# wwang2/CoarseGrainingVAE

Hardware: NVIDIA B200
Metric: conformations/s (fwd+bwd train step) (higher is better)
Workload: dtype f32

## Files before the change

### coarsegrainingvae_b200/_lib.py

```python
import ctypes
import os
import re

_HERE = os.path.dirname(os.path.abspath(__file__))
LIB_PATH = os.path.join(_HERE, "libcgvae_sm100.so")
HEADER_PATH = os.path.join(_HERE, "..", "include", "cgvae_b200.h")

_lib = None

_P = ctypes.c_void_p
_I64 = ctypes.c_int64
_INT = ctypes.c_int
_F32 = ctypes.c_float
_SZ = ctypes.c_size_t

SIGNATURES = {
    "cgvae_abi_version": (_INT, []),
    "cgvae_last_error": (ctypes.c_char_p, []),
    "cgvae_launch_count": (ctypes.c_ulonglong, []),
    "cgvae_set_error_flags": (_INT, [_INT, _P]),
    "cgvae_radius_graph_ws_bytes": (_SZ, [_I64, _I64]),
    "cgvae_radius_graph_count": (_INT, [_P, _I64, _P, _I64, _F32, _INT, _INT, _P, _P, _SZ, _P]),
    "cgvae_radius_graph_fill": (_INT, [_P, _I64, _P, _I64, _F32, _INT, _INT, _P, _P, _P, _SZ, _P]),
    "cgvae_exclusive_scan": (_INT, [_P, _I64, _P, _P]),
# ... 24 lines not shown
                                  _P, _P, _P, _P, _P, _P, _P, _P, _P, _P, _P]),
    "cgvae_update_norm_fwd": (_INT, [_P, _P, _I64, _INT, _P, _P]),
    "cgvae_update_combine_fwd": (_INT, [_P, _P, _P, _P, _P, _I64, _INT, _INT, _P, _P, _P]),
    "cgvae_update_combine_bwd": (_INT, [_P, _P, _P, _P, _P, _I64, _INT, _P, _P, _P, _P]),
    "cgvae_update_norm_bwd": (_INT, [_P, _P, _P, _P, _I64, _INT, _INT, _P, _P, _P]),
    "cgvae_update_combine_bwd_ld": (_INT, [_P, _P, _P, _P, _P, _I64, _INT, _P, _P, _P, _I64, _P]),
    "cgvae_update_norm_bwd_ld": (_INT, [_P, _P, _P, _P, _I64, _INT, _INT, _P, _P, _I64, _P]),
    "cgvae_segment_reduce_fwd": (_INT, [_P, _P, _P, _I64, _I64, _INT, _P, _P]),
    "cgvae_segment_reduce_bwd": (_INT, [_P, _P, _P, _I64, _I64, _INT, _P, _P]),
    "cgvae_gather_rows": (_INT, [_P, _P, _I64, _I64, _I64, _P, _P]),
    "cgvae_lift_fwd": (_INT, [_P, _P, _P, _P, _P, _P, _P, _I64, _I64, _INT, _INT, _P, _P]),
    "cgvae_lift_bwd": (_INT, [_P, _P, _P, _P, _P, _P, _I64, _I64, _INT, _INT, _P, _P]),
    "cgvae_adam_ws_bytes": (_SZ, []),
    "cgvae_adam_clip_step": (_INT, [_P, _P, _P, _P, _I64, _F32, _F32, _F32, _F32, _F32, _F32, _P, _P, _P, _F32, _F32, _P,
                                    _P, _SZ, _P]),
    "cgvae_bond_graph": (_INT, [_P, _P, _I64, _F32, _P, _P]),
    "cgvae_sample_quality": (_INT, [_P, _P, _P, _P, _I64, _I64, _F32, _P, _P, _P]),
    "cgvae_set_pdl": (_INT, [_INT]),
    "cgvae_set_matmul_precision": (_INT, [_INT]),
    "cgvae_get_matmul_precision": (_INT, []),
    "cgvae_register_const_range": (_INT, [_P, _SZ]),
    "cgvae_grad_sumsq": (_INT, [_P, _I64, _P, _P, _SZ, _P]),
    "cgvae_adam_apply": (_INT, [_P, _P, _P, _P, _I64, _F32, _F32, _F32, _F32, _F32, _F32, _P, _P, _INT, _F32, _F32, _P, _P, _SZ, _P]),
    "cgvae_dihedral_loss_fwd": (_INT, [_P, _P, _P, _I64, _P, _P, _P, _P, _P, _SZ, _P]),
    "cgvae_dihedral_loss_bwd": (_INT, [_P, _P, _P, _P, _I64, _I64, _P, _P, _P, _P]),
    "cgvae_pin_mask": (_INT, [_P, _I64, _P, _I64, _P, _SZ, _P]),
    "cgvae_vae_latent_fwd": (_INT, [_P, _P, _P, _I64, _P, _P, _P]),
    "cgvae_vae_latent_bwd": (_INT, [_P, _P, _P, _P, _I64, _P, _P, _P]),
    "cgvae_std_logvar_fwd": (_INT, [_P, _I64, _F32, _P, _P]),
    "cgvae_std_logvar_bwd": (_INT, [_P, _P, _I64, _F32, _P, _P]),
# ... 47 lines not shown
```

### coarsegrainingvae_b200/csrc/optim.cu

```cuda
#include "common.cuh"

namespace cgvae {

constexpr int kNormBlocks = 1024;

__global__ void __launch_bounds__(256) sumsq_partial_kernel(const float* __restrict__ g, int64_t n, float* __restrict__ partial,
                                                            unsigned int* __restrict__ ticket) {
  CGVAE_KERNEL_PROLOGUE();
  __shared__ float red[8];
  const int64_t per = (n + kNormBlocks - 1) / kNormBlocks;
  const int64_t beg = (int64_t)blockIdx.x * per, end = min(n, beg + per);
  float s = 0.f;
  for (int64_t i = beg + threadIdx.x; i < end; i += 256) {
    const float x = g[i];
    s = fmaf(x, x, s);
  }
  s = warp_sum(s);
  if ((threadIdx.x & 31) == 0) red[threadIdx.x >> 5] = s;
  __syncthreads();
  if (threadIdx.x == 0) {
    float t = 0.f;
#pragma unroll
    for (int w = 0; w < 8; ++w) t += red[w];
    partial[blockIdx.x] = t;
// ... 66 lines not shown
        const float gg = g[j] * coef;
        const float mm = beta1 * m[j] + (1.0f - beta1) * gg;
        const float vv = beta2 * v[j] + (1.0f - beta2) * gg * gg;
        m[j] = mm; v[j] = vv;
        p[j] -= step_size * mm / (sqrtf(vv) * inv_sqrt_bc2 + eps);
      }
    }
  }
  __syncthreads();
  if (threadIdx.x == 0) {
    __threadfence();
    if (atomicAdd(ticket, 1u) == gridDim.x - 1) step[0] = t;
  }
}

}

using namespace cgvae;

extern "C" {

size_t cgvae_adam_ws_bytes(void) { return sizeof(float) * (kNormBlocks + 4); }

int cgvae_adam_clip_step(float* p, const float* g, float* m, float* v, int64_t n, float max_norm, float grad_scale, float lr,
                         float beta1, float beta2, float eps, float* step, float* norm_out, const float* loss,
                         float loss_scale, float loss_limit, float* skipped, void* ws, size_t ws_bytes,
                         cgvae_stream_t stream) {
  if (n == 0) return 0;
  CGVAE_REQUIRE(p && g && m && v && step && ws && ws_bytes >= cgvae_adam_ws_bytes(), "adam_clip_step: bad arguments");
  CGVAE_REQUIRE(aligned16(p) && aligned16(g) && aligned16(m) && aligned16(v), "adam_clip_step: buffers must be 16-byte aligned");
// ... 21 lines not shown
int cgvae_adam_apply(float* p, const float* g, float* m, float* v, int64_t n, float max_norm, float grad_scale, float lr, float beta1,
                     float beta2, float eps, float* step, float* norm_out, int use_ws_loss, float loss_scale, float loss_limit,
                     float* skipped, void* ws, size_t ws_bytes, cgvae_stream_t stream) {
  if (n == 0) return 0;
  CGVAE_REQUIRE(p && g && m && v && step && ws && ws_bytes >= cgvae_adam_ws_bytes(), "adam_apply: bad arguments");
  CGVAE_REQUIRE(aligned16(p) && aligned16(g) && aligned16(m) && aligned16(v), "adam_apply: buffers must be 16-byte aligned");
  float* partial = reinterpret_cast<float*>(ws);
  unsigned int* ticket = reinterpret_cast<unsigned int*>(partial + kNormBlocks + 1);
  const unsigned blocks = (unsigned)std::min<int64_t>(ceil_div(n, 256 * 4), 148 * 8);
  launch_kernel(adam_clip_kernel, dim3(blocks), dim3(256), 0, (cudaStream_t)stream, p, g, m, v, n, (const float*)partial, max_norm, grad_scale, lr,
                beta1, beta2, eps, step, norm_out, use_ws_loss ? (const float*)(partial + kNormBlocks) : (const float*)nullptr, loss_scale,
                loss_limit, skipped, ticket);
  return launched("adam_clip");
}

}
```

### coarsegrainingvae_b200/csrc/wgrad.cu

```cuda
#include "common.cuh"

namespace cgvae {

constexpr int WG_MAXP = 48;
constexpr int WG_ROWS = 32;
constexpr int WG_T = 64;
constexpr int WG_STRIP = 4;
constexpr int WG_FAST_ROWS = 16;

struct WgradBatch {
  cgvae_wgrad_problem p[WG_MAXP];
  int tile_begin[WG_MAXP + 1];
  int n;
};
static_assert(sizeof(WgradBatch) <= 4000, "problem table must fit the 4 KB kernel parameter space");

__device__ __forceinline__ void stage_rows(float (*dst)[WG_T], const float* __restrict__ src, int ld, int r0, int rows,
                                           int c0, int ncols, bool vec, int tid, int seg_rows, int64_t seg_stride) {
  const int rn = min(WG_ROWS, rows - r0);
  for (int idx = tid; idx < rn * (WG_T / 4); idx += 256) {
    const int r = idx / (WG_T / 4), c = 4 * (idx % (WG_T / 4));
    float4 val = make_float4(0.f, 0.f, 0.f, 0.f);
    {
      const int R = r0 + r;
      const float* q;
      if (seg_rows > 0) {
        const int sgm = R / seg_rows;
        q = src + (int64_t)sgm * seg_stride + (int64_t)(R - sgm * seg_rows) * ld + c0 + c;
      } else {
        q = src + (int64_t)R * ld + c0 + c;
      }
      if (vec && c0 + c + 3 < ncols) {
        val = __ldg(reinterpret_cast<const float4*>(q));
      } else {
        if (c0 + c + 0 < ncols) val.x = __ldg(q + 0);
        if (c0 + c + 1 < ncols) val.y = __ldg(q + 1);
        if (c0 + c + 2 < ncols) val.z = __ldg(q + 2);
        if (c0 + c + 3 < ncols) val.w = __ldg(q + 3);
      }
    }
    *reinterpret_cast<float4*>(&dst[r][c]) = val;
  }
}

__global__ void __launch_bounds__(256) wgrad_grouped_kernel(const __grid_constant__ WgradBatch batch) {
  CGVAE_KERNEL_PROLOGUE();
  __shared__ __align__(16) float gs[WG_ROWS][WG_T];
  __shared__ __align__(16) float xs[WG_ROWS][WG_T];
  const int tid = threadIdx.x, bid = blockIdx.x;
  int lo = 0, hi = batch.n;
  while (hi - lo > 1) {
    const int mid = (lo + hi) >> 1;
    if (batch.tile_begin[mid] <= bid) lo = mid; else hi = mid;
  }
  const cgvae_wgrad_problem& P = batch.p[lo];
  const float* __restrict__ gy = P.gy;
  const float* __restrict__ x = P.x;
  float* __restrict__ dW = P.dW;
  float* __restrict__ db = P.db;
  const int rows = P.rows, n_out = P.n_out, n_in = P.n_in, ldg = P.ldg, ldx = P.ldx, seg_rows = P.seg_rows;
  const int64_t sg = P.seg_stride_g, sx = P.seg_stride_x;
  const bool has_w = (dW != nullptr);
  const int strips_k = has_w ? (n_in + WG_STRIP * WG_T - 1) / (WG_STRIP * WG_T) : 1;
  const int t = bid - batch.tile_begin[lo];
  const int n0 = (t / strips_k) * WG_T, kstrip = (t % strips_k) * WG_STRIP * WG_T;
  const bool g_vec = ((reinterpret_cast<uintptr_t>(gy) & 15) == 0) && (ldg % 4 == 0) && (seg_rows == 0 || sg % 4 == 0);
  const bool x_vec = has_w && ((reinterpret_cast<uintptr_t>(x) & 15) == 0) && (ldx % 4 == 0) && (seg_rows == 0 || sx % 4 == 0);
  const bool w_vec = has_w && ((reinterpret_cast<uintptr_t>(dW) & 15) == 0) && (n_in % 4 == 0);
  const int ty = tid >> 4, tx = tid & 15;
  const bool one_chunk = rows <= WG_ROWS;

  if (one_chunk) stage_rows(gs, gy, ldg, 0, rows, n0, n_out, g_vec, tid, seg_rows, sg);
  if (db != nullptr && kstrip == 0) {
    float bsum = 0.f;
    for (int r0 = 0; r0 < rows; r0 += WG_ROWS) {
      if (!one_chunk) {
        __syncthreads();
        stage_rows(gs, gy, ldg, r0, rows, n0, n_out, g_vec, tid, seg_rows, sg);
      }
      __syncthreads();
      const int rn = min(WG_ROWS, rows - r0);
      if (tid < WG_T)
        for (int r = 0; r < rn; ++r) bsum += gs[r][tid];
    }
    if (tid < WG_T && n0 + tid < n_out) db[n0 + tid] = bsum;
  }
  if (!has_w) return;
  if (rows <= WG_FAST_ROWS) {
    __shared__ __align__(16) float xw[WG_FAST_ROWS][WG_STRIP * WG_T];
    const int ncol4 = WG_STRIP * WG_T / 4;
    for (int idx = tid; idx < rows * ncol4; idx += 256) {
      const int r = idx / ncol4, c = 4 * (idx % ncol4);
      float4 val = make_float4(0.f, 0.f, 0.f, 0.f);
      const float* q;
      if (seg_rows > 0) {
        const int sgm = r / seg_rows;
        q = x + (int64_t)sgm * sx + (int64_t)(r - sgm * seg_rows) * ldx + kstrip + c;
      } else {
        q = x + (int64_t)r * ldx + kstrip + c;
      }
      if (x_vec && kstrip + c + 3 < n_in) {
        val = __ldg(reinterpret_cast<const float4*>(q));
      } else {
        if (kstrip + c + 0 < n_in) val.x = __ldg(q + 0);
        if (kstrip + c + 1 < n_in) val.y = __ldg(q + 1);
        if (kstrip + c + 2 < n_in) val.z = __ldg(q + 2);
        if (kstrip + c + 3 < n_in) val.w = __ldg(q + 3);
      }
      *reinterpret_cast<float4*>(&xw[r][c]) = val;
    }
    __syncthreads();
#pragma unroll
    for (int kk = 0; kk < WG_STRIP; ++kk) {
      const int k0 = kstrip + kk * WG_T;
      if (k0 >= n_in) break;
      float acc[4][4];
#pragma unroll
      for (int a = 0; a < 4; ++a)
#pragma unroll
        for (int b = 0; b < 4; ++b) acc[a][b] = 0.f;
      for (int r = 0; r < rows; ++r) {
        const float4 g4 = *reinterpret_cast<const float4*>(&gs[r][4 * ty]);
        const float4 x4 = *reinterpret_cast<const float4*>(&xw[r][kk * WG_T + 4 * tx]);
        const float g[4] = {g4.x, g4.y, g4.z, g4.w}, xv[4] = {x4.x, x4.y, x4.z, x4.w};
#pragma unroll
        for (int a = 0; a < 4; ++a)
#pragma unroll
          for (int b = 0; b < 4; ++b) acc[a][b] = fmaf(g[a], xv[b], acc[a][b]);
      }
      const int k = k0 + 4 * tx;
#pragma unroll
      for (int a = 0; a < 4; ++a) {
        const int n = n0 + 4 * ty + a;
        if (n >= n_out) continue;
        float* dst = dW + (int64_t)n * n_in + k;
        if (w_vec && k + 3 < n_in) {
          *reinterpret_cast<float4*>(dst) = make_float4(acc[a][0], acc[a][1], acc[a][2], acc[a][3]);
        } else {
#pragma unroll
          for (int b = 0; b < 4; ++b)
            if (k + b < n_in) dst[b] = acc[a][b];
        }
      }
    }
    return;
  }
  for (int kk = 0; kk < WG_STRIP; ++kk) {
    const int k0 = kstrip + kk * WG_T;
    if (k0 >= n_in) break;
    float acc[4][4];
#pragma unroll
    for (int a = 0; a < 4; ++a)
#pragma unroll
      for (int b = 0; b < 4; ++b) acc[a][b] = 0.f;
    for (int r0 = 0; r0 < rows; r0 += WG_ROWS) {
      __syncthreads();
      if (!one_chunk) stage_rows(gs, gy, ldg, r0, rows, n0, n_out, g_vec, tid, seg_rows, sg);
      stage_rows(xs, x, ldx, r0, rows, k0, n_in, x_vec, tid, seg_rows, sx);
      __syncthreads();
      const int rn = min(WG_ROWS, rows - r0);
#pragma unroll 4
      for (int r = 0; r < rn; ++r) {
        const float4 g4 = *reinterpret_cast<const float4*>(&gs[r][4 * ty]);
        const float4 x4 = *reinterpret_cast<const float4*>(&xs[r][4 * tx]);
        const float g[4] = {g4.x, g4.y, g4.z, g4.w}, xv[4] = {x4.x, x4.y, x4.z, x4.w};
#pragma unroll
        for (int a = 0; a < 4; ++a)
#pragma unroll
          for (int b = 0; b < 4; ++b) acc[a][b] = fmaf(g[a], xv[b], acc[a][b]);
      }
    }
    const int k = k0 + 4 * tx;
#pragma unroll
    for (int a = 0; a < 4; ++a) {
      const int n = n0 + 4 * ty + a;
      if (n >= n_out) continue;
      float* dst = dW + (int64_t)n * n_in + k;
      if (w_vec && k + 3 < n_in) {
        *reinterpret_cast<float4*>(dst) = make_float4(acc[a][0], acc[a][1], acc[a][2], acc[a][3]);
      } else {
#pragma unroll
        for (int b = 0; b < 4; ++b)
          if (k + b < n_in) dst[b] = acc[a][b];
      }
    }
  }
}

}

using namespace cgvae;

extern "C" {

int cgvae_wgrad_grouped(const cgvae_wgrad_problem* problems, int n_problems, cgvae_stream_t stream) {
  CGVAE_REQUIRE(n_problems >= 0, "wgrad_grouped: negative problem count");
  if (n_problems == 0) return 0;
  CGVAE_REQUIRE(problems != nullptr, "wgrad_grouped: null problem table");
  for (int i = 0; i < n_problems; ++i) {
    const cgvae_wgrad_problem& q = problems[i];
    CGVAE_REQUIRE(q.gy && (q.dW || q.db), "wgrad_grouped: problem %d has no operand / no output", i);
    CGVAE_REQUIRE(!q.dW || q.x, "wgrad_grouped: problem %d: dW without x", i);
    CGVAE_REQUIRE(q.rows >= 0 && q.n_out >= 1 && q.ldg >= q.n_out, "wgrad_grouped: problem %d: bad gy shape", i);
    CGVAE_REQUIRE(!q.dW || (q.n_in >= 1 && q.ldx >= q.n_in), "wgrad_grouped: problem %d: bad x shape", i);
    CGVAE_REQUIRE(q.seg_rows >= 0 && (q.seg_rows == 0 || q.rows % q.seg_rows == 0),
                  "wgrad_grouped: problem %d: rows must be a multiple of seg_rows", i);
  }
  cudaStream_t st = (cudaStream_t)stream;
  for (int base = 0; base < n_problems; base += WG_MAXP) {
    WgradBatch batch;
    batch.n = std::min(WG_MAXP, n_problems - base);
    int64_t tiles = 0;
    for (int i = 0; i < batch.n; ++i) {
      batch.p[i] = problems[base + i];
      batch.tile_begin[i] = (int)tiles;
      const cgvae_wgrad_problem& q = batch.p[i];
      tiles += ceil_div(q.n_out, WG_T) * (q.dW ? ceil_div(q.n_in, WG_STRIP * WG_T) : 1);
      CGVAE_REQUIRE(tiles < (int64_t)1 << 30, "wgrad_grouped: too many output tiles");
    }
    for (int i = batch.n; i <= WG_MAXP; ++i) batch.tile_begin[i] = (int)tiles;
    for (int i = batch.n; i < WG_MAXP; ++i) batch.p[i] = cgvae_wgrad_problem{};
    launch_kernel(wgrad_grouped_kernel, dim3((unsigned)tiles), dim3(256), 0, st, batch);
    if (int rc = launched("wgrad_grouped")) return rc;
  }
  return 0;
}

}
```

### coarsegrainingvae_b200/ops.py

```python
import contextlib as _contextlib

import numpy as np
import torch

from . import _lib

ACT_CODES = {None: 0, "none": 0, "linear": 0, "swish": 1, "ReLU": 2, "relu": 2, "Tanh": 3, "tanh": 3}
GEMM_NT, GEMM_NN, GEMM_TN = 0, 1, 2


def _p(t):
    if t is None:
        return None
    return t.data_ptr()


_raw_stream = torch._C._cuda_getCurrentRawStream if hasattr(torch._C, "_cuda_getCurrentRawStream") else None


def _stream():
    if _raw_stream is not None:
        return _raw_stream(torch.cuda.current_device())
    return torch.cuda.current_stream().cuda_stream

# ... 839 lines not shown
def adam_clip_step(p, g, m, v, step, max_norm, lr, betas=(0.9, 0.999), eps=1e-8, norm_out=None, grad_scale=1.0,
                   loss=None, loss_scale=1.0, loss_limit=float("inf"), skipped=None):
    _need_cuda(p, g, m, v, step)
    lib = _lib.load()
    ws_bytes = int(lib.cgvae_adam_ws_bytes())
    ws = torch.empty(ws_bytes, dtype=torch.uint8, device=p.device)
    t0 = TIMER.begin("adam_clip") if TIMER is not None else None
    _lib.check(lib.cgvae_adam_clip_step(_p(p), _p(g), _p(m), _p(v), p.numel(), float(max_norm), float(grad_scale), float(lr), float(betas[0]),
                                        float(betas[1]), float(eps), _p(step), _p(norm_out), _p(loss), float(loss_scale),
                                        float(min(loss_limit, 3.0e38)), _p(skipped), _p(ws), ws_bytes, _stream()),
               "adam_clip_step")
    if t0 is not None:
        TIMER.end("adam_clip", t0, dict(n=p.numel()))


def set_pdl(on):
    return bool(_lib.load().cgvae_set_pdl(int(bool(on))))


MATMUL_PRECISIONS = ("highest", "high")


def set_matmul_precision(mode):
    if mode not in MATMUL_PRECISIONS:
        raise ValueError("matmul precision must be one of %s, got %r" % (MATMUL_PRECISIONS, mode))
    rc = _lib.load().cgvae_set_matmul_precision(MATMUL_PRECISIONS.index(mode))
    if rc < 0:
        _lib.check(rc, "set_matmul_precision")
    return MATMUL_PRECISIONS[rc]

# ... 155 lines not shown
```

### coarsegrainingvae_b200/train.py

```python
import torch

EPS = 1e-6


def kl_divergence(mu1, std1, mu2, std2):
    if mu2 is None:
        return -0.5 * torch.sum(1 + torch.log(std1.pow(2)) - mu1.pow(2) - std1.pow(2), dim=-1).mean()
    return 0.5 * ((std1.pow(2) / std2.pow(2)).sum(-1) + ((mu1 - mu2).pow(2) / std2).sum(-1)
                  + torch.log(std2.pow(2)).sum(-1) - torch.log(std1.pow(2)).sum(-1) - std1.shape[-1]).mean()


def training_loss(outputs, xyz, bond_edge_list, beta, gamma, bond_count=None, norms=None):
    mu, sigma, pmu, pstd, _, xyz_recon = outputs
    if xyz_recon.is_cuda and FUSED_LOSS:
        return _training_loss_fused(outputs, xyz, bond_edge_list, beta, gamma, bond_count, norms)
    if norms is None:
        recon = (xyz_recon - xyz).pow(2).mean()
    else:
        recon = (xyz_recon - xyz).pow(2).sum() / (3.0 * norms[0])
    loss = recon
    kl = graph = None
    if mu is not None:
        kl = kl_divergence(mu, sigma, pmu, pstd)
        if norms is not None:
# ... 112 lines not shown
        self.flat = None
        self.opt = None
        self.flat_p = self.exp_avg = self.exp_avg_sq = self.step_count = None
        import os
        self.defer_grads = os.environ.get("CGVAE_DEFER_WGRAD", "1") != "0"
        self.gather_factors = os.environ.get("CGVAE_GATHER_FACTORS", "auto")
        self.dp_overlap = os.environ.get("CGVAE_DP_OVERLAP", "0") == "1"
        self.shard_opt = os.environ.get("CGVAE_SHARD_OPT", "auto")
        self._adam_ws = None
        self.n_overlap = 0
        self._comm_stream = None
        self._scope = None
        self.n_reduce = None
        self._arena = self._gathered = self._factor_table = None
        self._factor_layout = None

    def _loss(self, batch, eps):
        out = self.model(batch, eps=eps) if eps is not None else self.model(batch)
        xyz = out[4]
        return training_loss(out, xyz, batch["bond_edge_list"], self.beta, self.gamma, batch.get("bond_count"),
                             batch.get("dp_norms"))[0]

    def update_dp_norms(self, batch):
        import torch.distributed as dist
        world = self._world()
        if world == 1:
            return batch
        xyz = batch["nxyz"] if "nxyz" in batch else batch["xyz"]
        beads = batch["CG_nxyz"] if "CG_nxyz" in batch else batch["ca_xyz"]
        dev = xyz.device
# ... 66 lines not shown
            deferred_offsets = set()
            for _, _, dW, db in scope.pending:
                for t in (dW, db):
                    if t is not None:
                        deferred_offsets.add((t.data_ptr() - base) // 4)
            head, tail = [], []
            for p, (off, _) in zip(probe.params, probe.views):
                (tail if off in deferred_offsets else head).append(p)
        finally:
            probe.release()
            for p in params:
                p.grad = None
        self.n_reduce = sum(p.numel() for p in head)
        return head + tail

    def forward_backward(self, batch, eps=None):
        self.flat.zero_()
        loss = self._loss(batch, eps)
        if self.flat.sink and self.defer_grads:
            from . import ops
            if self.gather_factors:
                with ops.DeferredGrads(flush=False) as scope:
                    loss.backward()
                self._pack_factors(scope.pending)
            else:
                with ops.DeferredGrads() as scope:
                    self._scope = scope
                    self._arm_overlap()
                    try:
                        loss.backward()
                    finally:
                        self._scope = None
                        self.model._latent_grad_hook = None
        else:
            loss.backward()
        with torch.no_grad():
            self.flat.loss_slot.copy_(loss.detach().reshape(1))
        return loss

# ... 96 lines not shown
            guard = self.loss_limit is not None
            if self.shard_opt:
                import torch.distributed as dist
                world, r = self._world(), dist.get_rank(self.group)
                cnt = self.flat.n_padded // world
                g_sl, p_sl = self.flat.buffer[r * cnt:(r + 1) * cnt], self.flat_p[r * cnt:(r + 1) * cnt]
                if self._adam_ws is None:
                    self._adam_ws = ops.adam_ws(self.flat_p.device)
                ops.grad_sumsq(g_sl, self.flat.loss_slot if guard else None, self._adam_ws)
                dist.all_reduce(self._adam_ws[:1025], op=dist.ReduceOp.SUM, group=self.group)
                ops.adam_apply(p_sl, g_sl, self.exp_avg, self.exp_avg_sq, self.step_count, self.max_norm, self.lr, self._adam_ws,
                               grad_scale=1.0 / world, use_ws_loss=guard, loss_scale=1.0 / world,
                               loss_limit=self.loss_limit if guard else float("inf"), skipped=self.skipped)
                dist.all_gather_into_tensor(self.flat_p, p_sl, group=self.group)
                return
            ops.adam_clip_step(self.flat_p, self.flat.flat, self.exp_avg, self.exp_avg_sq, self.step_count, self.max_norm, self.lr,
                               grad_scale=1.0 / self._world(), loss=self.flat.loss_slot if guard else None,
                               loss_scale=1.0 / self._world(), loss_limit=self.loss_limit if guard else float("inf"),
                               skipped=self.skipped)
        else:
            if self.loss_limit is not None:
                l = float(self.flat.loss_slot.item())
                if l != l or l >= self.loss_limit:
                    self.n_skipped_host = getattr(self, "n_skipped_host", 0) + 1
                    return
            self.flat.clip_(self.max_norm)
            self.opt.step()

    def skipped_steps(self):
        n = getattr(self, "n_skipped_host", 0)
        if self.skipped is not None:
            n += int(self.skipped.item())
        return n

    def step(self, batch, eps=None, train=True):
        if self._world() > 1 and "dp_norms" not in batch and not torch.cuda.is_current_stream_capturing():
            batch = self.update_dp_norms(dict(batch))
        self._exchange_follows = bool(train)
        try:
            loss = self.forward_backward(batch, eps)
        finally:
            self._exchange_follows = False
        if train:
            self.exchange_gradients()
            self.apply_gradients()
        return loss


STATIC_LISTS = (("nbr_list", "nbr_count"), ("CG_nbr_list", "CG_nbr_count"), ("bond_edge_list", "bond_count"))


def compute_dihe(xyz, indices):
    b1 = xyz[indices[:, 1]] - xyz[indices[:, 0]]
    b2 = xyz[indices[:, 2]] - xyz[indices[:, 1]]
    b3 = xyz[indices[:, 3]] - xyz[indices[:, 2]]
    c1 = torch.linalg.cross(b2, b3)
    c2 = torch.linalg.cross(b1, b2)
# ... 311 lines not shown
```

### include/cgvae_b200.h

```cpp
#ifndef CGVAE_B200_H_
#define CGVAE_B200_H_

#include <stddef.h>
#include <stdint.h>

#ifdef __cplusplus
extern "C" {
#endif

typedef void* cgvae_stream_t;

#define CGVAE_ABI_VERSION 1

enum { CGVAE_ACT_NONE = 0, CGVAE_ACT_SWISH = 1, CGVAE_ACT_RELU = 2, CGVAE_ACT_TANH = 3,
       CGVAE_ACT_SIGMOID = 4, CGVAE_ACT_SHIFTED_SOFTPLUS = 5, CGVAE_ACT_LEAKY_RELU = 6, CGVAE_ACT_ELU = 7 };
enum { CGVAE_GEMM_NT = 0,
       CGVAE_GEMM_NN = 1,
       CGVAE_GEMM_TN = 2   };

int cgvae_abi_version(void);
const char* cgvae_last_error(void);
unsigned long long cgvae_launch_count(void);
enum { CGVAE_ERR_LIFT_RANK_BIT = 1,
       CGVAE_ERR_EMBED_INDEX_BIT = 2,
// ... 116 lines not shown
                      cgvae_stream_t stream);

int cgvae_lift_fwd(const float* V, const float* cg_xyz, const int64_t* mapping, const int64_t* rank,
                   const int32_t* rowptr_b, const int32_t* atoms, const uint8_t* pin, int64_t N, int64_t n_beads,
                   int F, int mode, float* xyz_out, cgvae_stream_t stream);
int cgvae_lift_bwd(const float* g_xyz, const int64_t* mapping, const int64_t* rank, const int32_t* rowptr_b,
                   const int32_t* atoms, const uint8_t* pin, int64_t N, int64_t n_beads, int F, int mode,
                   float* g_V, cgvae_stream_t stream);


size_t cgvae_adam_ws_bytes(void);
int cgvae_adam_clip_step(float* p, const float* g, float* m, float* v, int64_t n, float max_norm, float grad_scale,
                         float lr, float beta1, float beta2, float eps, float* step, float* norm_out,
                         const float* loss, float loss_scale, float loss_limit, float* skipped, void* ws,
                         size_t ws_bytes, cgvae_stream_t stream);
int cgvae_grad_sumsq(const float* g, int64_t n, const float* loss, void* ws, size_t ws_bytes, cgvae_stream_t stream);
int cgvae_adam_apply(float* p, const float* g, float* m, float* v, int64_t n, float max_norm, float grad_scale, float lr, float beta1,
                     float beta2, float eps, float* step, float* norm_out, int use_ws_loss, float loss_scale, float loss_limit,
                     float* skipped, void* ws, size_t ws_bytes, cgvae_stream_t stream);

int cgvae_vae_latent_fwd(const float* mu, const float* logvar, const float* eps, int64_t n, float* sigma, float* z,
                         cgvae_stream_t stream);
int cgvae_vae_latent_bwd(const float* g_z, const float* g_sigma, const float* eps, const float* sigma, int64_t n, float* g_mu,
                         float* g_logvar, cgvae_stream_t stream);
int cgvae_std_logvar_fwd(const float* x, int64_t n, float c, float* y, cgvae_stream_t stream);
int cgvae_std_logvar_bwd(const float* gy, const float* y, int64_t n, float c, float* gx, cgvae_stream_t stream);
size_t cgvae_loss_ws_bytes(void);
int cgvae_loss_fwd(const float* xyz, const float* xyz_rec, int64_t n_atoms, const int32_t* bond_rowptr, const int32_t* bond_col,
                   const float* mu, const float* sigma, const float* pmu, const float* pstd, int64_t n_beads, int F,
                   const float* norms, float beta, float gamma, float* out4, void* ws, size_t ws_bytes,
// ... 28 lines not shown
```

Measured before the change: 760.7.

## Fuse deferred weight-gradient GEMMs with gradient-norm reduction before Adam

Deferred weight-gradient problems are now handed to the optimizer, and a new kernel computes each dW/db strip while accumulating its squared norm in registers. The same kernel sums squares over the remaining plain gradient ranges, so the separate wgrad launch and the full reread of the gradient buffer for clipping go away. Adam then reads the combined partial sums. The cost is more host-side table building per step, a 32 KB parameter struct, and a workspace allocated on every call.

```diff
diff --git a/coarsegrainingvae_b200/_lib.py b/coarsegrainingvae_b200/_lib.py
--- a/coarsegrainingvae_b200/_lib.py
+++ b/coarsegrainingvae_b200/_lib.py
@@ -62,6 +62,8 @@
     "cgvae_adam_ws_bytes": (_SZ, []),
     "cgvae_adam_clip_step": (_INT, [_P, _P, _P, _P, _I64, _F32, _F32, _F32, _F32, _F32, _F32, _P, _P, _P, _F32, _F32, _P,
                                     _P, _SZ, _P]),
+    "cgvae_adam_clip_fused_step": (_INT, [_P, _P, _P, _P, _I64, _P, _INT, _F32, _F32, _F32, _F32, _F32, _F32, _P, _P, _P,
+                                          _F32, _F32, _P, _P, _SZ, _P]),
     "cgvae_bond_graph": (_INT, [_P, _P, _I64, _F32, _P, _P]),
     "cgvae_sample_quality": (_INT, [_P, _P, _P, _P, _I64, _I64, _F32, _P, _P, _P]),
     "cgvae_set_pdl": (_INT, [_INT]),
diff --git a/coarsegrainingvae_b200/csrc/optim.cu b/coarsegrainingvae_b200/csrc/optim.cu
--- a/coarsegrainingvae_b200/csrc/optim.cu
+++ b/coarsegrainingvae_b200/csrc/optim.cu
@@ -1,4 +1,8 @@
-#include "common.cuh"
+#include <algorithm>
+#include <utility>
+#include <vector>
+
+#include "wgrad_strip.cuh"
 
 namespace cgvae {
 
@@ -104,6 +108,91 @@
   }
 }
 
+constexpr int FA_MAXP = 192;
+constexpr int FA_MAXR = FA_MAXP + 1;
+constexpr int FA_CHUNK = 4096;
+
+struct FusedBatch {
+  cgvae_wgrad_problem p[FA_MAXP];
+  int64_t r_beg[FA_MAXR], r_end[FA_MAXR];
+  int item_begin[FA_MAXP + FA_MAXR + 1];
+  int np, nr;
+};
+static_assert(sizeof(FusedBatch) <= 32000, "problem table must fit the 32 KB kernel parameter space");
+
+__device__ __forceinline__ int fused_entry(const FusedBatch& b, int w) {
+  int lo = 0, hi = b.np + b.nr;
+  while (hi - lo > 1) {
+    const int mid = (lo + hi) >> 1;
+    if (b.item_begin[mid] <= w) lo = mid; else hi = mid;
+  }
+  return lo;
+}
+
+struct StoreSumsq {
+  float s;
+  __device__ __forceinline__ void bias(float* dst, float val) {
+    *dst = val;
+    s = fmaf(val, val, s);
+  }
+  __device__ __forceinline__ void tile(float* __restrict__ dW, int n_first, int n_out, int k, int n_in, bool w_vec,
+                                       const float (&acc)[4][4]) {
+    WgradStore().tile(dW, n_first, n_out, k, n_in, w_vec, acc);
+#pragma unroll
+    for (int a = 0; a < 4; ++a)
+#pragma unroll
+      for (int b = 0; b < 4; ++b)
+        if (n_first + a < n_out && k + b < n_in) s = fmaf(acc[a][b], acc[a][b], s);
+  }
+};
+
+__global__ void __launch_bounds__(256) adam_clip_wgrad_sumsq_kernel(const __grid_constant__ FusedBatch batch, const float* __restrict__ g,
+                                                          float* __restrict__ partial, int first, unsigned int* __restrict__ ticket) {
+  CGVAE_KERNEL_PROLOGUE();
+  __shared__ WgradSmem sm;
+  __shared__ float red[8];
+  StoreSumsq out{0.f};
+  const int items = batch.item_begin[batch.np + batch.nr];
+  for (int w = blockIdx.x; w < items; w += gridDim.x) {
+    const int e = fused_entry(batch, w);
+    const int t = w - batch.item_begin[e];
+    if (e < batch.np) {
+      __syncthreads();
+      wgrad_strip(batch.p[e], t, sm, out);
+    } else {
+      const int64_t beg = batch.r_beg[e - batch.np] + (int64_t)t * FA_CHUNK;
+      const int64_t end = min(batch.r_end[e - batch.np], beg + FA_CHUNK);
+      for (int64_t i = beg + threadIdx.x; i < end; i += 256) {
+        const float x = g[i];
+        out.s = fmaf(x, x, out.s);
+      }
+    }
+  }
+  float s = warp_sum(out.s);
+  if ((threadIdx.x & 31) == 0) red[threadIdx.x >> 5] = s;
+  __syncthreads();
+  if (threadIdx.x == 0) {
+    float t = 0.f;
+#pragma unroll
+    for (int w = 0; w < 8; ++w) t += red[w];
+    partial[blockIdx.x] = first ? t : partial[blockIdx.x] + t;
+    if (first) {
+      for (int i = blockIdx.x + gridDim.x; i < kNormBlocks; i += gridDim.x) partial[i] = 0.f;
+      if (blockIdx.x == 0) *ticket = 0u;
+    }
+  }
+}
+
+static int fused_blocks_per_sm() {
+  static int n = 0;
+  if (n == 0) {
+    int a = 0;
+    if (cudaOccupancyMaxActiveBlocksPerMultiprocessor(&a, adam_clip_wgrad_sumsq_kernel, 256, 0) != cudaSuccess) return 1;
+    n = std::max(1, a);
+  }
+  return n;
+}
+
 }
 
 using namespace cgvae;
@@ -155,4 +244,82 @@
   return launched("adam_clip");
 }
 
-}
+int cgvae_adam_clip_fused_step(float* p, float* g, float* m, float* v, int64_t n, const cgvae_wgrad_problem* problems,
+                               int n_problems, float max_norm, float grad_scale, float lr, float beta1, float beta2, float eps,
+                               float* step, float* norm_out, const float* loss, float loss_scale, float loss_limit,
+                               float* skipped, void* ws, size_t ws_bytes, cgvae_stream_t stream) {
+  if (n == 0) return 0;
+  CGVAE_REQUIRE(p && g && m && v && step && ws && ws_bytes >= cgvae_adam_ws_bytes(), "adam_clip_fused_step: bad arguments");
+  CGVAE_REQUIRE(aligned16(p) && aligned16(g) && aligned16(m) && aligned16(v),
+                "adam_clip_fused_step: buffers must be 16-byte aligned");
+  CGVAE_REQUIRE(n_problems >= 0 && (n_problems == 0 || problems != nullptr), "adam_clip_fused_step: bad problem table");
+  std::vector<std::pair<int64_t, int64_t>> out;
+  for (int i = 0; i < n_problems; ++i) {
+    const cgvae_wgrad_problem& q = problems[i];
+    CGVAE_REQUIRE(q.gy && (q.dW || q.db), "adam_clip_fused_step: problem %d has no operand / no output", i);
+    CGVAE_REQUIRE(!q.dW || q.x, "adam_clip_fused_step: problem %d: dW without x", i);
+    CGVAE_REQUIRE(q.rows >= 0 && q.n_out >= 1 && q.ldg >= q.n_out, "adam_clip_fused_step: problem %d: bad gy shape", i);
+    CGVAE_REQUIRE(!q.dW || (q.n_in >= 1 && q.ldx >= q.n_in), "adam_clip_fused_step: problem %d: bad x shape", i);
+    CGVAE_REQUIRE(q.seg_rows >= 0 && (q.seg_rows == 0 || q.rows % q.seg_rows == 0),
+                  "adam_clip_fused_step: problem %d: rows must be a multiple of seg_rows", i);
+    const float* o[2] = {q.dW, q.db};
+    const int64_t len[2] = {(int64_t)q.n_out * q.n_in, q.n_out};
+    for (int j = 0; j < 2; ++j) {
+      if (!o[j]) continue;
+      const int64_t b = o[j] - g;
+      CGVAE_REQUIRE(o[j] >= g && b + len[j] <= n, "adam_clip_fused_step: problem %d: output outside the gradient buffer", i);
+      out.emplace_back(b, b + len[j]);
+    }
+  }
+  std::sort(out.begin(), out.end());
+  std::vector<std::pair<int64_t, int64_t>> plain;
+  int64_t pos = 0;
+  for (const auto& r : out) {
+    CGVAE_REQUIRE(r.first >= pos, "adam_clip_fused_step: problem outputs overlap");
+    if (r.first > pos) plain.emplace_back(pos, r.first);
+    pos = r.second;
+  }
+  if (pos < n) plain.emplace_back(pos, n);
+
+  const int np = n_problems, nr = (int)plain.size();
+  const int n_batches = (int)std::max(ceil_div(np, FA_MAXP), ceil_div(nr, FA_MAXR));
+  std::vector<FusedBatch> batches(n_batches);
+  std::vector<int> items(n_batches);
+  for (int k = 0; k < n_batches; ++k) {
+    FusedBatch& b = batches[k];
+    b = FusedBatch{};
+    b.np = std::max(0, std::min(FA_MAXP, np - k * FA_MAXP));
+    b.nr = std::max(0, std::min(FA_MAXR, nr - k * FA_MAXR));
+    int64_t it = 0;
+    for (int i = 0; i < b.np; ++i) {
+      b.p[i] = problems[k * FA_MAXP + i];
+      b.item_begin[i] = (int)it;
+      it += wgrad_strips(b.p[i]);
+    }
+    for (int i = 0; i < b.nr; ++i) {
+      b.r_beg[i] = plain[k * FA_MAXR + i].first;
+      b.r_end[i] = plain[k * FA_MAXR + i].second;
+      b.item_begin[b.np + i] = (int)it;
+      it += ceil_div(b.r_end[i] - b.r_beg[i], FA_CHUNK);
+      CGVAE_REQUIRE(it < (int64_t)1 << 30, "adam_clip_fused_step: too many work items");
+    }
+    b.item_begin[b.np + b.nr] = (int)it;
+    items[k] = (int)it;
+  }
+
+  cudaStream_t st = (cudaStream_t)stream;
+  float* partial = reinterpret_cast<float*>(ws);
+  unsigned int* ticket = reinterpret_cast<unsigned int*>(partial + kNormBlocks + 1);
+  const int resident = kNumSM * fused_blocks_per_sm();
+  for (int k = 0; k < n_batches; ++k) {
+    const unsigned blocks = (unsigned)std::max(1, std::min({items[k], resident, kNormBlocks}));
+    launch_kernel(adam_clip_wgrad_sumsq_kernel, dim3(blocks), dim3(256), 0, st, batches[k], (const float*)g, partial, k == 0 ? 1 : 0, ticket);
+    if (int rc = launched("adam_clip_wgrad_sumsq")) return rc;
+  }
+  const unsigned blocks = (unsigned)std::min<int64_t>(ceil_div(n, 256 * 4), 148 * 8);
+  launch_kernel(adam_clip_kernel, dim3(blocks), dim3(256), 0, st, p, (const float*)g, m, v, n, (const float*)partial, max_norm, grad_scale,
+                lr, beta1, beta2, eps, step, norm_out, loss, loss_scale, loss_limit, skipped, ticket);
+  return launched("adam_clip");
+}
+
+}
diff --git a/coarsegrainingvae_b200/csrc/wgrad.cu b/coarsegrainingvae_b200/csrc/wgrad.cu
--- a/coarsegrainingvae_b200/csrc/wgrad.cu
+++ b/coarsegrainingvae_b200/csrc/wgrad.cu
@@ -1,12 +1,8 @@
-#include "common.cuh"
+#include "wgrad_strip.cuh"
 
 namespace cgvae {
 
 constexpr int WG_MAXP = 48;
-constexpr int WG_ROWS = 32;
-constexpr int WG_T = 64;
-constexpr int WG_STRIP = 4;
-constexpr int WG_FAST_ROWS = 16;
 
 struct WgradBatch {
   cgvae_wgrad_problem p[WG_MAXP];
@@ -15,176 +11,17 @@
 };
 static_assert(sizeof(WgradBatch) <= 4000, "problem table must fit the 4 KB kernel parameter space");
 
-__device__ __forceinline__ void stage_rows(float (*dst)[WG_T], const float* __restrict__ src, int ld, int r0, int rows,
-                                           int c0, int ncols, bool vec, int tid, int seg_rows, int64_t seg_stride) {
-  const int rn = min(WG_ROWS, rows - r0);
-  for (int idx = tid; idx < rn * (WG_T / 4); idx += 256) {
-    const int r = idx / (WG_T / 4), c = 4 * (idx % (WG_T / 4));
-    float4 val = make_float4(0.f, 0.f, 0.f, 0.f);
-    {
-      const int R = r0 + r;
-      const float* q;
-      if (seg_rows > 0) {
-        const int sgm = R / seg_rows;
-        q = src + (int64_t)sgm * seg_stride + (int64_t)(R - sgm * seg_rows) * ld + c0 + c;
-      } else {
-        q = src + (int64_t)R * ld + c0 + c;
-      }
-      if (vec && c0 + c + 3 < ncols) {
-        val = __ldg(reinterpret_cast<const float4*>(q));
-      } else {
-        if (c0 + c + 0 < ncols) val.x = __ldg(q + 0);
-        if (c0 + c + 1 < ncols) val.y = __ldg(q + 1);
-        if (c0 + c + 2 < ncols) val.z = __ldg(q + 2);
-        if (c0 + c + 3 < ncols) val.w = __ldg(q + 3);
-      }
-    }
-    *reinterpret_cast<float4*>(&dst[r][c]) = val;
-  }
-}
-
 __global__ void __launch_bounds__(256) wgrad_grouped_kernel(const __grid_constant__ WgradBatch batch) {
   CGVAE_KERNEL_PROLOGUE();
-  __shared__ __align__(16) float gs[WG_ROWS][WG_T];
-  __shared__ __align__(16) float xs[WG_ROWS][WG_T];
-  const int tid = threadIdx.x, bid = blockIdx.x;
+  __shared__ WgradSmem sm;
+  const int bid = blockIdx.x;
   int lo = 0, hi = batch.n;
   while (hi - lo > 1) {
     const int mid = (lo + hi) >> 1;
     if (batch.tile_begin[mid] <= bid) lo = mid; else hi = mid;
   }
-  const cgvae_wgrad_problem& P = batch.p[lo];
-  const float* __restrict__ gy = P.gy;
-  const float* __restrict__ x = P.x;
-  float* __restrict__ dW = P.dW;
-  float* __restrict__ db = P.db;
-  const int rows = P.rows, n_out = P.n_out, n_in = P.n_in, ldg = P.ldg, ldx = P.ldx, seg_rows = P.seg_rows;
-  const int64_t sg = P.seg_stride_g, sx = P.seg_stride_x;
-  const bool has_w = (dW != nullptr);
-  const int strips_k = has_w ? (n_in + WG_STRIP * WG_T - 1) / (WG_STRIP * WG_T) : 1;
-  const int t = bid - batch.tile_begin[lo];
-  const int n0 = (t / strips_k) * WG_T, kstrip = (t % strips_k) * WG_STRIP * WG_T;
-  const bool g_vec = ((reinterpret_cast<uintptr_t>(gy) & 15) == 0) && (ldg % 4 == 0) && (seg_rows == 0 || sg % 4 == 0);
-  const bool x_vec = has_w && ((reinterpret_cast<uintptr_t>(x) & 15) == 0) && (ldx % 4 == 0) && (seg_rows == 0 || sx % 4 == 0);
-  const bool w_vec = has_w && ((reinterpret_cast<uintptr_t>(dW) & 15) == 0) && (n_in % 4 == 0);
-  const int ty = tid >> 4, tx = tid & 15;
-  const bool one_chunk = rows <= WG_ROWS;
-
-  if (one_chunk) stage_rows(gs, gy, ldg, 0, rows, n0, n_out, g_vec, tid, seg_rows, sg);
-  if (db != nullptr && kstrip == 0) {
-    float bsum = 0.f;
-    for (int r0 = 0; r0 < rows; r0 += WG_ROWS) {
-      if (!one_chunk) {
-        __syncthreads();
-        stage_rows(gs, gy, ldg, r0, rows, n0, n_out, g_vec, tid, seg_rows, sg);
-      }
-      __syncthreads();
-      const int rn = min(WG_ROWS, rows - r0);
-      if (tid < WG_T)
-        for (int r = 0; r < rn; ++r) bsum += gs[r][tid];
-    }
-    if (tid < WG_T && n0 + tid < n_out) db[n0 + tid] = bsum;
-  }
-  if (!has_w) return;
-  if (rows <= WG_FAST_ROWS) {
-    __shared__ __align__(16) float xw[WG_FAST_ROWS][WG_STRIP * WG_T];
-    const int ncol4 = WG_STRIP * WG_T / 4;
-    for (int idx = tid; idx < rows * ncol4; idx += 256) {
-      const int r = idx / ncol4, c = 4 * (idx % ncol4);
-      float4 val = make_float4(0.f, 0.f, 0.f, 0.f);
-      const float* q;
-      if (seg_rows > 0) {
-        const int sgm = r / seg_rows;
-        q = x + (int64_t)sgm * sx + (int64_t)(r - sgm * seg_rows) * ldx + kstrip + c;
-      } else {
-        q = x + (int64_t)r * ldx + kstrip + c;
-      }
-      if (x_vec && kstrip + c + 3 < n_in) {
-        val = __ldg(reinterpret_cast<const float4*>(q));
-      } else {
-        if (kstrip + c + 0 < n_in) val.x = __ldg(q + 0);
-        if (kstrip + c + 1 < n_in) val.y = __ldg(q + 1);
-        if (kstrip + c + 2 < n_in) val.z = __ldg(q + 2);
-        if (kstrip + c + 3 < n_in) val.w = __ldg(q + 3);
-      }
-      *reinterpret_cast<float4*>(&xw[r][c]) = val;
-    }
-    __syncthreads();
-#pragma unroll
-    for (int kk = 0; kk < WG_STRIP; ++kk) {
-      const int k0 = kstrip + kk * WG_T;
-      if (k0 >= n_in) break;
-      float acc[4][4];
-#pragma unroll
-      for (int a = 0; a < 4; ++a)
-#pragma unroll
-        for (int b = 0; b < 4; ++b) acc[a][b] = 0.f;
-      for (int r = 0; r < rows; ++r) {
-        const float4 g4 = *reinterpret_cast<const float4*>(&gs[r][4 * ty]);
-        const float4 x4 = *reinterpret_cast<const float4*>(&xw[r][kk * WG_T + 4 * tx]);
-        const float g[4] = {g4.x, g4.y, g4.z, g4.w}, xv[4] = {x4.x, x4.y, x4.z, x4.w};
-#pragma unroll
-        for (int a = 0; a < 4; ++a)
-#pragma unroll
-          for (int b = 0; b < 4; ++b) acc[a][b] = fmaf(g[a], xv[b], acc[a][b]);
-      }
-      const int k = k0 + 4 * tx;
-#pragma unroll
-      for (int a = 0; a < 4; ++a) {
-        const int n = n0 + 4 * ty + a;
-        if (n >= n_out) continue;
-        float* dst = dW + (int64_t)n * n_in + k;
-        if (w_vec && k + 3 < n_in) {
-          *reinterpret_cast<float4*>(dst) = make_float4(acc[a][0], acc[a][1], acc[a][2], acc[a][3]);
-        } else {
-#pragma unroll
-          for (int b = 0; b < 4; ++b)
-            if (k + b < n_in) dst[b] = acc[a][b];
-        }
-      }
-    }
-    return;
-  }
-  for (int kk = 0; kk < WG_STRIP; ++kk) {
-    const int k0 = kstrip + kk * WG_T;
-    if (k0 >= n_in) break;
-    float acc[4][4];
-#pragma unroll
-    for (int a = 0; a < 4; ++a)
-#pragma unroll
-      for (int b = 0; b < 4; ++b) acc[a][b] = 0.f;
-    for (int r0 = 0; r0 < rows; r0 += WG_ROWS) {
-      __syncthreads();
-      if (!one_chunk) stage_rows(gs, gy, ldg, r0, rows, n0, n_out, g_vec, tid, seg_rows, sg);
-      stage_rows(xs, x, ldx, r0, rows, k0, n_in, x_vec, tid, seg_rows, sx);
-      __syncthreads();
-      const int rn = min(WG_ROWS, rows - r0);
-#pragma unroll 4
-      for (int r = 0; r < rn; ++r) {
-        const float4 g4 = *reinterpret_cast<const float4*>(&gs[r][4 * ty]);
-        const float4 x4 = *reinterpret_cast<const float4*>(&xs[r][4 * tx]);
-        const float g[4] = {g4.x, g4.y, g4.z, g4.w}, xv[4] = {x4.x, x4.y, x4.z, x4.w};
-#pragma unroll
-        for (int a = 0; a < 4; ++a)
-#pragma unroll
-          for (int b = 0; b < 4; ++b) acc[a][b] = fmaf(g[a], xv[b], acc[a][b]);
-      }
-    }
-    const int k = k0 + 4 * tx;
-#pragma unroll
-    for (int a = 0; a < 4; ++a) {
-      const int n = n0 + 4 * ty + a;
-      if (n >= n_out) continue;
-      float* dst = dW + (int64_t)n * n_in + k;
-      if (w_vec && k + 3 < n_in) {
-        *reinterpret_cast<float4*>(dst) = make_float4(acc[a][0], acc[a][1], acc[a][2], acc[a][3]);
-      } else {
-#pragma unroll
-        for (int b = 0; b < 4; ++b)
-          if (k + b < n_in) dst[b] = acc[a][b];
-      }
-    }
-  }
+  WgradStore out;
+  wgrad_strip(batch.p[lo], bid - batch.tile_begin[lo], sm, out);
 }
 
 }
@@ -215,7 +52,7 @@
       batch.p[i] = problems[base + i];
       batch.tile_begin[i] = (int)tiles;
       const cgvae_wgrad_problem& q = batch.p[i];
-      tiles += ceil_div(q.n_out, WG_T) * (q.dW ? ceil_div(q.n_in, WG_STRIP * WG_T) : 1);
+      tiles += wgrad_strips(q);
       CGVAE_REQUIRE(tiles < (int64_t)1 << 30, "wgrad_grouped: too many output tiles");
     }
     for (int i = batch.n; i <= WG_MAXP; ++i) batch.tile_begin[i] = (int)tiles;
diff --git a/coarsegrainingvae_b200/csrc/wgrad_strip.cuh b/coarsegrainingvae_b200/csrc/wgrad_strip.cuh
--- /dev/null
+++ b/coarsegrainingvae_b200/csrc/wgrad_strip.cuh
@@ -0,0 +1,184 @@
+#pragma once
+#include "common.cuh"
+
+namespace cgvae {
+
+constexpr int WG_ROWS = 32;
+constexpr int WG_T = 64;
+constexpr int WG_STRIP = 4;
+constexpr int WG_FAST_ROWS = 16;
+
+struct WgradSmem {
+  __align__(16) float gs[WG_ROWS][WG_T];
+  union {
+    __align__(16) float xs[WG_ROWS][WG_T];
+    __align__(16) float xw[WG_FAST_ROWS][WG_STRIP * WG_T];
+  };
+};
+
+__host__ __device__ inline int wgrad_strips(const cgvae_wgrad_problem& q) {
+  return ((q.n_out + WG_T - 1) / WG_T) * (q.dW ? (q.n_in + WG_STRIP * WG_T - 1) / (WG_STRIP * WG_T) : 1);
+}
+
+__device__ __forceinline__ void stage_rows(float (*dst)[WG_T], const float* __restrict__ src, int ld, int r0, int rows,
+                                           int c0, int ncols, bool vec, int tid, int seg_rows, int64_t seg_stride) {
+  const int rn = min(WG_ROWS, rows - r0);
+  for (int idx = tid; idx < rn * (WG_T / 4); idx += 256) {
+    const int r = idx / (WG_T / 4), c = 4 * (idx % (WG_T / 4));
+    float4 val = make_float4(0.f, 0.f, 0.f, 0.f);
+    {
+      const int R = r0 + r;
+      const float* q;
+      if (seg_rows > 0) {
+        const int sgm = R / seg_rows;
+        q = src + (int64_t)sgm * seg_stride + (int64_t)(R - sgm * seg_rows) * ld + c0 + c;
+      } else {
+        q = src + (int64_t)R * ld + c0 + c;
+      }
+      if (vec && c0 + c + 3 < ncols) {
+        val = __ldg(reinterpret_cast<const float4*>(q));
+      } else {
+        if (c0 + c + 0 < ncols) val.x = __ldg(q + 0);
+        if (c0 + c + 1 < ncols) val.y = __ldg(q + 1);
+        if (c0 + c + 2 < ncols) val.z = __ldg(q + 2);
+        if (c0 + c + 3 < ncols) val.w = __ldg(q + 3);
+      }
+    }
+    *reinterpret_cast<float4*>(&dst[r][c]) = val;
+  }
+}
+
+template <class Out>
+__device__ __forceinline__ void wgrad_strip(const cgvae_wgrad_problem& P, int t, WgradSmem& sm, Out& out) {
+  const int tid = threadIdx.x;
+  const float* __restrict__ gy = P.gy;
+  const float* __restrict__ x = P.x;
+  float* __restrict__ dW = P.dW;
+  float* __restrict__ db = P.db;
+  const int rows = P.rows, n_out = P.n_out, n_in = P.n_in, ldg = P.ldg, ldx = P.ldx, seg_rows = P.seg_rows;
+  const int64_t sg = P.seg_stride_g, sx = P.seg_stride_x;
+  const bool has_w = (dW != nullptr);
+  const int strips_k = has_w ? (n_in + WG_STRIP * WG_T - 1) / (WG_STRIP * WG_T) : 1;
+  const int n0 = (t / strips_k) * WG_T, kstrip = (t % strips_k) * WG_STRIP * WG_T;
+  const bool g_vec = ((reinterpret_cast<uintptr_t>(gy) & 15) == 0) && (ldg % 4 == 0) && (seg_rows == 0 || sg % 4 == 0);
+  const bool x_vec = has_w && ((reinterpret_cast<uintptr_t>(x) & 15) == 0) && (ldx % 4 == 0) && (seg_rows == 0 || sx % 4 == 0);
+  const bool w_vec = has_w && ((reinterpret_cast<uintptr_t>(dW) & 15) == 0) && (n_in % 4 == 0);
+  const int ty = tid >> 4, tx = tid & 15;
+  const bool one_chunk = rows <= WG_ROWS;
+  float (*gs)[WG_T] = sm.gs;
+  float (*xs)[WG_T] = sm.xs;
+
+  if (one_chunk) stage_rows(gs, gy, ldg, 0, rows, n0, n_out, g_vec, tid, seg_rows, sg);
+  if (db != nullptr && kstrip == 0) {
+    float bsum = 0.f;
+    for (int r0 = 0; r0 < rows; r0 += WG_ROWS) {
+      if (!one_chunk) {
+        __syncthreads();
+        stage_rows(gs, gy, ldg, r0, rows, n0, n_out, g_vec, tid, seg_rows, sg);
+      }
+      __syncthreads();
+      const int rn = min(WG_ROWS, rows - r0);
+      if (tid < WG_T)
+        for (int r = 0; r < rn; ++r) bsum += gs[r][tid];
+    }
+    if (tid < WG_T && n0 + tid < n_out) out.bias(db + n0 + tid, bsum);
+  }
+  if (!has_w) return;
+  if (rows <= WG_FAST_ROWS) {
+    float (*xw)[WG_STRIP * WG_T] = sm.xw;
+    const int ncol4 = WG_STRIP * WG_T / 4;
+    for (int idx = tid; idx < rows * ncol4; idx += 256) {
+      const int r = idx / ncol4, c = 4 * (idx % ncol4);
+      float4 val = make_float4(0.f, 0.f, 0.f, 0.f);
+      const float* q;
+      if (seg_rows > 0) {
+        const int sgm = r / seg_rows;
+        q = x + (int64_t)sgm * sx + (int64_t)(r - sgm * seg_rows) * ldx + kstrip + c;
+      } else {
+        q = x + (int64_t)r * ldx + kstrip + c;
+      }
+      if (x_vec && kstrip + c + 3 < n_in) {
+        val = __ldg(reinterpret_cast<const float4*>(q));
+      } else {
+        if (kstrip + c + 0 < n_in) val.x = __ldg(q + 0);
+        if (kstrip + c + 1 < n_in) val.y = __ldg(q + 1);
+        if (kstrip + c + 2 < n_in) val.z = __ldg(q + 2);
+        if (kstrip + c + 3 < n_in) val.w = __ldg(q + 3);
+      }
+      *reinterpret_cast<float4*>(&xw[r][c]) = val;
+    }
+    __syncthreads();
+#pragma unroll
+    for (int kk = 0; kk < WG_STRIP; ++kk) {
+      const int k0 = kstrip + kk * WG_T;
+      if (k0 >= n_in) break;
+      float acc[4][4];
+#pragma unroll
+      for (int a = 0; a < 4; ++a)
+#pragma unroll
+        for (int b = 0; b < 4; ++b) acc[a][b] = 0.f;
+      for (int r = 0; r < rows; ++r) {
+        const float4 g4 = *reinterpret_cast<const float4*>(&gs[r][4 * ty]);
+        const float4 x4 = *reinterpret_cast<const float4*>(&xw[r][kk * WG_T + 4 * tx]);
+        const float g[4] = {g4.x, g4.y, g4.z, g4.w}, xv[4] = {x4.x, x4.y, x4.z, x4.w};
+#pragma unroll
+        for (int a = 0; a < 4; ++a)
+#pragma unroll
+          for (int b = 0; b < 4; ++b) acc[a][b] = fmaf(g[a], xv[b], acc[a][b]);
+      }
+      const int k = k0 + 4 * tx;
+      if (k < n_in) out.tile(dW, n0 + 4 * ty, n_out, k, n_in, w_vec, acc);
+    }
+    return;
+  }
+  for (int kk = 0; kk < WG_STRIP; ++kk) {
+    const int k0 = kstrip + kk * WG_T;
+    if (k0 >= n_in) break;
+    float acc[4][4];
+#pragma unroll
+    for (int a = 0; a < 4; ++a)
+#pragma unroll
+      for (int b = 0; b < 4; ++b) acc[a][b] = 0.f;
+    for (int r0 = 0; r0 < rows; r0 += WG_ROWS) {
+      __syncthreads();
+      if (!one_chunk) stage_rows(gs, gy, ldg, r0, rows, n0, n_out, g_vec, tid, seg_rows, sg);
+      stage_rows(xs, x, ldx, r0, rows, k0, n_in, x_vec, tid, seg_rows, sx);
+      __syncthreads();
+      const int rn = min(WG_ROWS, rows - r0);
+#pragma unroll 4
+      for (int r = 0; r < rn; ++r) {
+        const float4 g4 = *reinterpret_cast<const float4*>(&gs[r][4 * ty]);
+        const float4 x4 = *reinterpret_cast<const float4*>(&xs[r][4 * tx]);
+        const float g[4] = {g4.x, g4.y, g4.z, g4.w}, xv[4] = {x4.x, x4.y, x4.z, x4.w};
+#pragma unroll
+        for (int a = 0; a < 4; ++a)
+#pragma unroll
+          for (int b = 0; b < 4; ++b) acc[a][b] = fmaf(g[a], xv[b], acc[a][b]);
+      }
+    }
+    const int k = k0 + 4 * tx;
+    if (k < n_in) out.tile(dW, n0 + 4 * ty, n_out, k, n_in, w_vec, acc);
+  }
+}
+
+struct WgradStore {
+  __device__ __forceinline__ void bias(float* dst, float val) { *dst = val; }
+  __device__ __forceinline__ void tile(float* __restrict__ dW, int n_first, int n_out, int k, int n_in, bool w_vec,
+                                       const float (&acc)[4][4]) {
+#pragma unroll
+    for (int a = 0; a < 4; ++a) {
+      const int n = n_first + a;
+      if (n >= n_out) continue;
+      float* dst = dW + (int64_t)n * n_in + k;
+      if (w_vec && k + 3 < n_in) {
+        *reinterpret_cast<float4*>(dst) = make_float4(acc[a][0], acc[a][1], acc[a][2], acc[a][3]);
+      } else {
+#pragma unroll
+        for (int b = 0; b < 4; ++b)
+          if (k + b < n_in) dst[b] = acc[a][b];
+      }
+    }
+  }
+};
+
+}
diff --git a/coarsegrainingvae_b200/ops.py b/coarsegrainingvae_b200/ops.py
--- a/coarsegrainingvae_b200/ops.py
+++ b/coarsegrainingvae_b200/ops.py
@@ -877,6 +877,23 @@
         TIMER.end("adam_clip", t0, dict(n=p.numel()))
 
 
+def adam_clip_fused_step(p, g, m, v, step, problems, max_norm, lr, betas=(0.9, 0.999), eps=1e-8, norm_out=None, grad_scale=1.0,
+                         loss=None, loss_scale=1.0, loss_limit=float("inf"), skipped=None):
+    _need_cuda(p, g, m, v, step)
+    lib = _lib.load()
+    table = wgrad_table(problems)
+    ws_bytes = int(lib.cgvae_adam_ws_bytes())
+    ws = torch.empty(ws_bytes, dtype=torch.uint8, device=p.device)
+    t0 = TIMER.begin("adam_clip") if TIMER is not None else None
+    _lib.check(lib.cgvae_adam_clip_fused_step(_p(p), _p(g), _p(m), _p(v), p.numel(), table.ctypes.data, len(table), float(max_norm),
+                                              float(grad_scale), float(lr), float(betas[0]), float(betas[1]), float(eps), _p(step),
+                                              _p(norm_out), _p(loss), float(loss_scale), float(min(loss_limit, 3.0e38)), _p(skipped),
+                                              _p(ws), ws_bytes, _stream()),
+               "adam_clip_fused_step")
+    if t0 is not None:
+        TIMER.end("adam_clip", t0, dict(n=p.numel(), problems=len(table)))
+
+
 def set_pdl(on):
     return bool(_lib.load().cgvae_set_pdl(int(bool(on))))
 
diff --git a/coarsegrainingvae_b200/train.py b/coarsegrainingvae_b200/train.py
--- a/coarsegrainingvae_b200/train.py
+++ b/coarsegrainingvae_b200/train.py
@@ -150,6 +150,8 @@
         self.n_reduce = None
         self._arena = self._gathered = self._factor_table = None
         self._factor_layout = None
+        self._defer_to_optimizer = False
+        self._pending = None
 
     def _loss(self, batch, eps):
         out = self.model(batch, eps=eps) if eps is not None else self.model(batch)
@@ -246,8 +248,13 @@
         self.n_reduce = sum(p.numel() for p in head)
         return head + tail
 
+    def _fuse_deferred(self):
+        return (self.flat_p is not None and self.defer_grads and self._world() == 1 and not self.shard_opt
+                and not self.n_overlap and not self.gather_factors)
+
     def forward_backward(self, batch, eps=None):
         self.flat.zero_()
+        self._pending = None
         loss = self._loss(batch, eps)
         if self.flat.sink and self.defer_grads:
             from . import ops
@@ -255,6 +262,10 @@
                 with ops.DeferredGrads(flush=False) as scope:
                     loss.backward()
                 self._pack_factors(scope.pending)
+            elif self._defer_to_optimizer:
+                with ops.DeferredGrads(flush=False) as scope:
+                    loss.backward()
+                self._pending = scope.pending
             else:
                 with ops.DeferredGrads() as scope:
                     self._scope = scope
@@ -381,6 +392,12 @@
                                loss_limit=self.loss_limit if guard else float("inf"), skipped=self.skipped)
                 dist.all_gather_into_tensor(self.flat_p, p_sl, group=self.group)
                 return
+            pending, self._pending = self._pending, None
+            if pending:
+                ops.adam_clip_fused_step(self.flat_p, self.flat.flat, self.exp_avg, self.exp_avg_sq, self.step_count, pending,
+                                         self.max_norm, self.lr, loss=self.flat.loss_slot if guard else None,
+                                         loss_limit=self.loss_limit if guard else float("inf"), skipped=self.skipped)
+                return
             ops.adam_clip_step(self.flat_p, self.flat.flat, self.exp_avg, self.exp_avg_sq, self.step_count, self.max_norm, self.lr,
                                grad_scale=1.0 / self._world(), loss=self.flat.loss_slot if guard else None,
                                loss_scale=1.0 / self._world(), loss_limit=self.loss_limit if guard else float("inf"),
@@ -404,10 +421,11 @@
         if self._world() > 1 and "dp_norms" not in batch and not torch.cuda.is_current_stream_capturing():
             batch = self.update_dp_norms(dict(batch))
         self._exchange_follows = bool(train)
+        self._defer_to_optimizer = bool(train) and self._fuse_deferred()
         try:
             loss = self.forward_backward(batch, eps)
         finally:
-            self._exchange_follows = False
+            self._exchange_follows = self._defer_to_optimizer = False
         if train:
             self.exchange_gradients()
             self.apply_gradients()
diff --git a/include/cgvae_b200.h b/include/cgvae_b200.h
--- a/include/cgvae_b200.h
+++ b/include/cgvae_b200.h
@@ -154,6 +154,10 @@
                          float lr, float beta1, float beta2, float eps, float* step, float* norm_out,
                          const float* loss, float loss_scale, float loss_limit, float* skipped, void* ws,
                          size_t ws_bytes, cgvae_stream_t stream);
+int cgvae_adam_clip_fused_step(float* p, float* g, float* m, float* v, int64_t n, const cgvae_wgrad_problem* problems,
+                               int n_problems, float max_norm, float grad_scale, float lr, float beta1, float beta2, float eps,
+                               float* step, float* norm_out, const float* loss, float loss_scale, float loss_limit,
+                               float* skipped, void* ws, size_t ws_bytes, cgvae_stream_t stream);
 int cgvae_grad_sumsq(const float* g, int64_t n, const float* loss, void* ws, size_t ws_bytes, cgvae_stream_t stream);
 int cgvae_adam_apply(float* p, const float* g, float* m, float* v, int64_t n, float max_norm, float grad_scale, float lr, float beta1,
                      float beta2, float eps, float* step, float* norm_out, int use_ws_loss, float loss_scale, float loss_limit,
```

New measurement: 762.5 (median of 6 runs). About the same (+0.2%).
